# pabloconrat/our_first_climate_model

Measured on NVIDIA B200. Metric: column*wavelength*layer flux updates/s (repwvl-100 RCE step), higher is better.
Workload: dtype f64

## Files before the change

our_first_climate_model_b200/csrc/rcm_capi.cu:

```cuda
#include <algorithm>
#include <cmath>
#include <cstdio>
#include <cstdlib>
#include <cstring>
#include <new>
#include <functional>
#include <string>
#include <vector>

#include "rcm_jac.cuh"
#include "rcm_fdh.cuh"
#include "rcm_lbl_diag.cuh"

#ifndef M_PI
#define M_PI 3.14159265358979323846
#endif

struct rcm_solver {
    int device = 0;
    cudaStream_t own_stream = nullptr, stream = nullptr;
    rcm_params p{};
    DevConst dc{};
    bool const_dirty = true;
    int opt_angle_cubes = 1;
// ... 421 lines not shown
}


bool use_split(const rcm_solver* s) {
    return !s->lbl_mode && s->has_table && s->nactive == 5 && s->opt_config == 0 && s->opt_path == 0;
}

struct SplitGeom { int ntiles, nitem, nsplit; };
SplitGeom split_geom(const rcm_solver* s, int ncols) {
    SplitGeom g;
    g.ntiles = (ncols + 15) / 16;
    g.nitem = (s->dc.nwvl + 3) / 4;
    g.nsplit = (g.nitem + rcm_split_ipu() - 1) / rcm_split_ipu();
    return g;
}

int ensure_split(rcm_solver* s) {
    const SplitGeom g = split_geom(s, s->cap);
    const size_t tiles = (size_t)g.ntiles, need_part = tiles * g.nsplit * rcm_split_part_doubles();
    if (tiles > s->tile_cap || !s->d_tile) {
        CU(dalloc(s->d_tile, tiles * rcm_split_tile_bytes()));
        s->tile_cap = tiles;
        s->tile_vmr_valid = false;
    }
    if (need_part > s->spart_cap || !s->d_spart) {
        CU(dalloc(s->d_spart, need_part));
        s->spart_cap = need_part;
    }
    if (tiles > s->multi_cap || !s->d_multi) {
        if (s->d_multi) CU(cudaFree(s->d_multi));
        s->d_multi = nullptr;
        CU(cudaMalloc((void**)&s->d_multi, 2 * tiles * sizeof(unsigned)));
        s->multi_cap = tiles;
    }
    if (!s->d_dTstat) CU(dalloc(s->d_dTstat, (size_t)s->cap));
    if (!s->d_counter) {
        CU(dalloc(s->d_counter, (size_t)4));
        CU(cudaMemsetAsync(s->d_counter, 0, 4 * sizeof(unsigned), s->stream));
    }
    return RCM_OK;
}

SplitArgs split_args(rcm_solver* s, int col0, int ncols, int which) {
    const SplitGeom g = split_geom(s, ncols);
    const size_t o = (size_t)col0, t0 = o / 16;
    SplitArgs a{};
    a.ncol = ncols;
    a.diag_ncol = s->ncol;
    a.ntiles = g.ntiles;
    a.nsplit = g.nsplit;
    a.ipu = rcm_split_ipu();
    a.nitem = g.nitem;
    a.nunits = g.ntiles * g.nsplit;
    a.stage_rows = s->opt_stage_rows;
    a.clampk = s->clampk;
    a.h2o_slot = s->h2o_slot;
    a.tau_clamp = s->tau_clamp;
    a.T_floor = s->T_floor;
    a.coef = s->d_coef3;
    a.planck_c = s->d_planck_c;
    a.planck_k = s->d_planck_k;
    a.exp_tab = s->d_exp_tab;
    a.Tlayer = s->d_T + o * NLAY;
    a.Tsurf = s->d_Ts + o;
    a.vmr = s->d_vmr + o * s->nactive * NLAY;
    a.rel_hum = s->d_rh + o * NLAY;
    a.Tprev = s->d_Tprev + o * NLAY;
    a.time_h = s->d_time + o;
    a.E_down = s->d_Ed + o * NLEV;
    a.E_up = s->d_Eu + o * NLEV;
    a.dE = s->d_dE + o * NLAY;
    a.dt = s->d_dt + o;
    a.diag = s->d_diag + o * 4;
    a.solar_col = s->has_col_solar ? s->d_solar_col + o : nullptr;
    a.cloud_col = s->has_col_cloud ? s->d_cloud_col + o : nullptr;
    a.tile = s->d_tile + t0 * rcm_split_tile_bytes();
    a.part = s->d_spart + t0 * g.nsplit * rcm_split_part_doubles();
    a.dTstat = s->d_dTstat + o;
    a.counter = s->d_counter + which;
    a.quota = 1 << 30;
    return a;
}

int split_grid(const rcm_solver* s, const SplitArgs& a, int nsm) {
    (void)s;
    if (a.quota < a.nunits) return (a.nunits + a.quota - 1) / a.quota;
    int per_sm = 3;
    if (const char* e = std::getenv("RCM_CTAS_PER_SM")) {
        const int v = std::atoi(e);
        if (v >= 1 && v < per_sm) per_sm = v;
    }
    return std::min(a.nunits, nsm * per_sm);
}

int split_rt(rcm_solver* s, const SplitArgs& a, int nsm, cudaStream_t st, bool timed) {
    std::pair<cudaEvent_t, cudaEvent_t> ev{};
    if (timed) {
        if (!s->ev_free.empty()) {
            ev = s->ev_free.back();
            s->ev_free.pop_back();
        } else {
            CU(cudaEventCreate(&ev.first));
            CU(cudaEventCreate(&ev.second));
        }
        CU(cudaEventRecord(ev.first, st));
    }
    CU(rcm_launch_split_rt(a, split_grid(s, a, nsm), st));
    s->launches += 1;
    if (timed) {
        CU(cudaEventRecord(ev.second, st));
        s->ev_used.push_back(ev);
        if (s->ev_used.size() >= 1024) {
            const int rc = rcm_kernel_time_ms(s, 0, nullptr, nullptr);
            if (rc != RCM_OK) return rc;
        }
    }
    return RCM_OK;
}

int split_advance(rcm_solver* s, int nsteps) {
    int st = refresh_const(s);
    if (st != RCM_OK) return st;
    st = ensure_split(s);
    if (st != RCM_OK) return st;
    const int nsm = nsm_of(s);
    const SplitArgs a = split_args(s, 0, s->ncol, 0);
    SplitColFlags f{};
    f.prep = 1;
    f.first = (s->step_index == 0);
    f.write_all_vmr = !s->tile_vmr_valid;
    CU(rcm_launch_split_col(a, f, s->stream));
    s->launches += 1;
    s->tile_vmr_valid = true;
    static const int multi_rounds = std::getenv("RCM_MULTI_ROUNDS") ? std::atoi(std::getenv("RCM_MULTI_ROUNDS")) : 24;
    const int grid1 = split_grid(s, a, nsm);
    const bool few_rounds = a.nunits < (long long)multi_rounds * grid1;
    const bool fits = (long long)a.nunits * nsteps + 2LL * grid1 < (1LL << 31);
    if (nsteps >= 2 && fits && (s->opt_multi == 2 || (s->opt_multi == 1 && few_rounds))) {
        SplitMultiArgs m{};
        m.nsteps = nsteps;
        m.done = s->d_multi;
        m.ready = s->d_multi + a.ntiles;
        CU(cudaMemsetAsync(s->d_multi, 0, 2 * (size_t)a.ntiles * sizeof(unsigned), s->stream));
        SplitArgs am = a;
        am.quota = 1 << 30;
        CU(rcm_launch_split_multi(am, m, split_grid(s, am, nsm), s->stream));
        s->launches += 1;
        return RCM_OK;
    }
    for (int k = 0; k < nsteps; ++k) {
        st = split_rt(s, a, nsm, s->stream, k < 4);
        if (st != RCM_OK) return st;
        SplitColFlags e{};
        e.finish = 1;
        e.prep = (k + 1 < nsteps);
        e.first = 0;
        e.write_out = (k + 1 == nsteps);
        e.diag_step = k;
        CU(rcm_launch_split_col(a, e, s->stream));
        s->launches += 1;
    }
    return RCM_OK;
}

int launch(rcm_solver* s, int mode, int nsteps, bool want_diag) {
    int st = refresh_const(s);
    if (st != RCM_OK) return st;
    if (mode == MODE_RT ? !s->has_spectral : !s->has_table) return fail(s, RCM_ERR_STATE, "no lookup table loaded");
    if (s->ncol <= 0) return fail(s, RCM_ERR_STATE, "no columns loaded");
    const int nsm = nsm_of(s);
    Part parts[2];
    const int nparts = plan_parts(s, s->ncol, nsm, parts);
    std::pair<cudaEvent_t, cudaEvent_t> ev;
    if (!s->ev_free.empty()) {
        ev = s->ev_free.back();
        s->ev_free.pop_back();
    } else {
        CU(cudaEventCreate(&ev.first));
        CU(cudaEventCreate(&ev.second));
    }
    CU(cudaEventRecord(ev.first, s->stream));
    for (int ip = 0; ip < nparts; ++ip) {
        st = launch_part(s, mode, nsteps, want_diag, parts[ip], nsm, s->stream);
        if (st != RCM_OK) return st;
    }
    CU(cudaEventRecord(ev.second, s->stream));
    if (mode == MODE_STEP) s->ev_used.push_back(ev); else s->ev_free.push_back(ev);
    if (s->ev_used.size() >= 1024) {
        st = rcm_kernel_time_ms(s, 0, nullptr, nullptr);
        if (st != RCM_OK) return st;
    }
    return RCM_OK;
}


int step_host_split(rcm_solver* s, int nchunk, const double* Tlayer_in, const double* Tsurf_in, const double* vmr_active_in,
                    double* E_down, double* E_up, double* dE, double* Tlayer_out, double* Tsurf_out) {
    int st = ensure_split(s);
    if (st != RCM_OK) return st;
    if (!s->sp_up) {
        int lo = 0, hi = 0;
        CU(cudaDeviceGetStreamPriorityRange(&lo, &hi));
        CU(cudaStreamCreateWithPriority(&s->sp_up, cudaStreamNonBlocking, hi));
        CU(cudaStreamCreateWithPriority(&s->sp_down, cudaStreamNonBlocking, hi));
        for (int i = 0; i < 2; ++i) CU(cudaStreamCreateWithPriority(&s->sp_rt[i], cudaStreamNonBlocking, lo));
        for (int i = 0; i < 24; ++i) {
            CU(cudaEventCreateWithFlags(&s->sp_prep[i], cudaEventDisableTiming));
            CU(cudaEventCreateWithFlags(&s->sp_rtdone[i], cudaEventDisableTiming));
        }
        CU(cudaEventCreateWithFlags(&s->sp_end, cudaEventDisableTiming));
    }
    const int nsm = nsm_of(s);
    const int per = ((s->ncol + nchunk - 1) / nchunk + 15) / 16 * 16;
    int bounds[24];
    int nb = 0;
    bounds[nb++] = 0;
    if (nchunk >= 4 && per >= 64) {
        const int q = per / 4 / 16 * 16;
        bounds[nb++] = q;
        for (int c0 = per; c0 < s->ncol - q; c0 += per) bounds[nb++] = c0;
        bounds[nb++] = std::max(bounds[nb - 1], s->ncol - q) / 16 * 16;
    } else {
        for (int c0 = per; c0 < s->ncol; c0 += per) bounds[nb++] = c0;
    }
    bounds[nb] = s->ncol;
    const size_t D = sizeof(double);
    const int na = s->nactive;
    auto enqueue = [&](bool timed) -> int {
    int nk = 0;
// ... 1510 lines not shown
```

our_first_climate_model_b200/csrc/rcm_kernels.cu:

```cuda
#include <cfloat>
#include <cstdio>

#include "rcm_kernels.cuh"
#include "rcm_diag.cuh"
#include "rcm_jac.cuh"
#include "rcm_fjac.cuh"
#include "rcm_fdh.cuh"
#include "rcm_lbl_diag.cuh"

__constant__ DevConst cst;

cudaError_t rcm_upload_const(const DevConst& c) { return cudaMemcpyToSymbol(cst, &c, sizeof(DevConst)); }

namespace {

#include "rcm_device_math.cuh"
#include "rcm_step_kernel.cuh"

__global__ void rcm_coef_kernel(const double* __restrict__ src, double* __restrict__ dst, int nt, int ns, int nw,
                                int np, int nact, const int* __restrict__ species) {
    const size_t n = (size_t)NLAY * (nt - 1) * nw * nact;
    for (size_t i = blockIdx.x * (size_t)blockDim.x + threadIdx.x; i < n; i += (size_t)gridDim.x * blockDim.x) {
        size_t r = i;
        const int k = r % nact; r /= nact;
// ... 156 lines not shown
    for (int k = 0; k < a.doublings; ++k) {
        const double denom = sub(1.0, mul(r, r));
        const double r2 = add(r, dvd(mul(mul(r, t), t), denom));
        const double t2 = dvd(mul(t, t), denom);
        const double s2 = add(dvd(add(mul(t, s_dir), mul(mul(mul(t_dir, r_dir), r), t)), denom), mul(t_dir, s_dir));
        const double rd2 = add(dvd(add(mul(mul(t, s_dir), r), mul(mul(t, t_dir), r)), denom), r_dir);
        t_dir = mul(t_dir, t_dir);
        s_dir = s2;
        r_dir = rd2;
        r = r2;
        t = t2;
    }
    const double r_total = add(r_dir, mul(mul(dvd(add(t_dir, s_dir), sub(1.0, mul(albedo, r))), t), albedo));
    if (a.r_total) a.r_total[i] = r_total;
    if (a.solar_irr) a.solar_irr[i] = mul(mul(mul(a.daytime, a.E_0), mu_s), sub(1.0, r_total));
    if (a.cloud_tau) a.cloud_tau[i] = dvd(tau_s, 2.0);
}

__global__ void __launch_bounds__(256) rcm_cplkavg_kernel(int n, const double* lo, const double* hi, const double* t,
                                                          double* out, const double* tab, int narrow) {
    __shared__ double stab[EXP_TAB * EXP_REP];
    for (int i = threadIdx.x; i < EXP_TAB * EXP_REP; i += blockDim.x) stab[i] = tab[i / EXP_REP];
    __syncthreads();
    const unsigned tl = (unsigned)__cvta_generic_to_shared(stab + (threadIdx.x & (EXP_REP - 1)));
    for (int i = blockIdx.x * blockDim.x + threadIdx.x; i < n; i += gridDim.x * blockDim.x)
    {
        const double whi = 1.0E7 / lo[i], wlo = 1.0E7 / hi[i];
        const bool bin_ok = whi > wlo && wlo >= 0. && (whi - wlo) / whi < 1.e-2;
        out[i] = narrow ? cplkavg_narrow(lo[i], hi[i], whi, wlo, bin_ok, t[i], tl) : cplkavg_dev(lo[i], hi[i], t[i]);
    }
}

}

size_t rcm_step_smem_bytes(int C, int nactive, int nthreads) {
#define RCM_SHAPE(CC, TT) \
    if (C == CC && nthreads == TT) return nactive == 5 ? Smem<CC, TT, 5>::bytes(5) : Smem<CC, TT, 0>::bytes(nactive);
    RCM_SHAPE(16, 128)
    RCM_SHAPE(8, 128)
    RCM_SHAPE(4, 128)
    RCM_SHAPE(32, 192)
    RCM_SHAPE(16, 96)
#undef RCM_SHAPE
    return 0;
}

template <int MODE, int NACT, int C, int NT>
static cudaError_t launch_t(const StepArgs& a, int nactive, int grid, cudaStream_t st) {
    const size_t smem = Smem<C, NT, NACT>::bytes(nactive);
    auto kern = a.clampk ? rcm_step_kernel<MODE, NACT, C, NT, true> : rcm_step_kernel<MODE, NACT, C, NT, false>;
    cudaError_t e = cudaFuncSetAttribute(kern, cudaFuncAttributeMaxDynamicSharedMemorySize, (int)smem);
    if (e != cudaSuccess) return e;
    kern<<<grid, NT, smem, st>>>(a);
    return cudaGetLastError();
}

template <int MODE>
static cudaError_t launch_m(const StepArgs& a, int nactive, int grid, cudaStream_t st) {
    const bool five = (nactive == 5);
#define RCM_SHAPE(CC, TT)                  \
    if (a.C == CC && a.nthreads == TT)     \
        return five ? launch_t<MODE, 5, CC, TT>(a, nactive, grid, st) : launch_t<MODE, 0, CC, TT>(a, nactive, grid, st);
    RCM_SHAPE(16, 128)
    RCM_SHAPE(8, 128)
    RCM_SHAPE(4, 128)
    RCM_SHAPE(32, 192)
    RCM_SHAPE(16, 96)
#undef RCM_SHAPE
    return cudaErrorInvalidValue;
}

cudaError_t rcm_launch_step(int mode, const StepArgs& a, int nactive, int grid, cudaStream_t st) {
    switch (mode) {
        case MODE_STEP: return launch_m<MODE_STEP>(a, nactive, grid, st);
        case MODE_TAU: return launch_m<MODE_TAU>(a, nactive, grid, st);
        case MODE_RT: return launch_m<MODE_RT>(a, nactive, grid, st);
    }
    return cudaErrorInvalidValue;
}

size_t rcm_split_tile_bytes() { return TILE_BYTES; }
size_t rcm_split_part_doubles() { return SPLIT_PART; }
int rcm_split_ipu() { return SPLIT_IPU; }

cudaError_t rcm_launch_split_col(const SplitArgs& a, const SplitColFlags& f, cudaStream_t st) {
    rcm_split_col_kernel<<<a.ntiles, SPLIT_COL_NT, 0, st>>>(a, f);
    return cudaGetLastError();
}

cudaError_t rcm_launch_split_rt(const SplitArgs& a, int grid, cudaStream_t st) {
    auto kern = a.clampk ? rcm_split_rt_kernel<true> : rcm_split_rt_kernel<false>;
    cudaError_t e = cudaFuncSetAttribute(kern, cudaFuncAttributeMaxDynamicSharedMemorySize, (int)SPLIT_SMEM);
    if (e != cudaSuccess) return e;
    kern<<<grid, SPLIT_NT, SPLIT_SMEM, st>>>(a);
    return cudaGetLastError();
}

cudaError_t rcm_launch_split_multi(const SplitArgs& a, const SplitMultiArgs& m, int grid, cudaStream_t st) {
    auto kern = a.clampk ? rcm_split_multi_kernel<true> : rcm_split_multi_kernel<false>;
    cudaError_t e = cudaFuncSetAttribute(kern, cudaFuncAttributeMaxDynamicSharedMemorySize, (int)SPLIT_SMEM);
    if (e != cudaSuccess) return e;
    kern<<<grid, SPLIT_NT, SPLIT_SMEM, st>>>(a, m);
    return cudaGetLastError();
}

size_t rcm_reduce_scratch_doubles(int nsteps) { return (size_t)nsteps * RED_BLOCKS * 4; }

cudaError_t rcm_launch_reduce_diag(const double* diag, int nsteps, int ncol, double dT_converged, double* scratch,
                                   unsigned* ticket, double* scalars, cudaStream_t st) {
    rcm_reduce_diag_kernel<<<dim3(RED_BLOCKS, nsteps), RED_THREADS, 0, st>>>(diag, ncol, dT_converged, scratch, ticket, scalars);
    return cudaGetLastError();
}

cudaError_t rcm_launch_coef(const double* xsec_file, double* coef, int nt, int ns, int nw, int np, int nact,
                            const int* d_species, cudaStream_t st) {
    rcm_coef_kernel<<<296, 256, 0, st>>>(xsec_file, coef, nt, ns, nw, np, nact, d_species);
    return cudaGetLastError();
}

cudaError_t rcm_launch_coef3(const double* coef4, double* coef3, size_t nrows, cudaStream_t st) {
    rcm_coef3_kernel<<<296, 256, 0, st>>>(coef4, coef3, nrows);
    return cudaGetLastError();
}

cudaError_t rcm_launch_microbench(int which, double* out, const double* tab, long iters, int grid,
                                  cudaStream_t st) {
    switch (which) {
        case 0: rcm_microbench_kernel<0><<<grid, 256, 0, st>>>(out, iters, tab); break;
        case 1: rcm_microbench_kernel<1><<<grid, 256, 0, st>>>(out, iters, tab); break;
        case 2: rcm_microbench_kernel<2><<<grid, 256, 0, st>>>(out, iters, tab); break;
        case 3: rcm_microbench_kernel<3><<<grid, 256, 0, st>>>(out, iters, tab); break;
        default: return cudaErrorInvalidValue;
    }
    return cudaGetLastError();
}

cudaError_t rcm_launch_solar(const SolarArgs& a, cudaStream_t st) {
    if (a.n <= 0) return cudaSuccess;
    rcm_solar_kernel<<<(a.n + 127) / 128, 128, 0, st>>>(a);
    return cudaGetLastError();
}

cudaError_t rcm_launch_cplkavg(int n, const double* lo, const double* hi, const double* t, double* out,
                               const double* exp_tab, int narrow, cudaStream_t st) {
    rcm_cplkavg_kernel<<<148, 256, 0, st>>>(n, lo, hi, t, out, exp_tab, narrow);
    return cudaGetLastError();
}

size_t rcm_lbl_smem_bytes(int C, int nthreads) {
    return ((size_t)EXP_TAB * EXP_REP + (size_t)TBD_LEN * 3 + 2 * C + (size_t)HALF * nthreads +
            (size_t)NLEV * (nthreads / 2)) * sizeof(double);
}

cudaError_t rcm_launch_lbl_prep(const LblArgs& a, cudaStream_t st) {
    rcm_lbl_prep_kernel<<<(a.ncol + 127) / 128, 128, 0, st>>>(a);
    return cudaGetLastError();
}

cudaError_t rcm_launch_lbl_rt(const LblArgs& a, cudaStream_t st, cudaEvent_t ev0, cudaEvent_t ev1) {
    constexpr int C = RCM_LBL_C, NT = RCM_LBL_NT;
    const size_t smem = rcm_lbl_smem_bytes(C, NT);
    auto kern = a.clampk ? rcm_lbl_rt_kernel<C, NT, true> : rcm_lbl_rt_kernel<C, NT, false>;
    cudaError_t e = cudaFuncSetAttribute(kern, cudaFuncAttributeMaxDynamicSharedMemorySize, (int)smem);
    if (e != cudaSuccess) return e;
    if (ev0) cudaEventRecord(ev0, st);
    kern<<<a.ntiles * a.nchunks, NT, smem, st>>>(a);
    if (ev1) cudaEventRecord(ev1, st);
    return cudaGetLastError();
}

cudaError_t rcm_launch_lbl_finish(const LblArgs& a, cudaStream_t st) {
    rcm_lbl_finish_kernel<<<a.ncol, LBL_FIN_NT, 0, st>>>(a);
    return cudaGetLastError();
}

cudaError_t rcm_launch_lbl_step(const LblArgs& a, cudaStream_t st, cudaEvent_t ev0, cudaEvent_t ev1) {
    cudaError_t e = rcm_launch_lbl_prep(a, st);
// ... 97 lines not shown
```

our_first_climate_model_b200/csrc/rcm_kernels.cuh:

```cuda
#ifndef RCM_KERNELS_CUH
#define RCM_KERNELS_CUH

#include <cuda_runtime.h>

#include "rcm_internal.h"

constexpr int NLAY = RCM_NLAYER;
constexpr int NLEV = RCM_NLEVEL;
constexpr int MAX_ANGLE = 64;
constexpr int MAX_TPERT = 16;
constexpr int PLK_MAX = 128;
constexpr int MAX_PAIR = 16;
constexpr int HALF = NLAY / 2;
constexpr int RCM_LBL_C = 16, RCM_LBL_NT = 128;
#ifndef RCM_EXP_LOG2
#define RCM_EXP_LOG2 10
#endif
constexpr int EXP_LOG2 = RCM_EXP_LOG2, EXP_TAB = 1 << EXP_LOG2;
constexpr int EXP_REP = (EXP_LOG2 == 7) ? 8 : 1;
#ifdef RCM_EXP_DEG_OVERRIDE
constexpr int EXP_DEG = RCM_EXP_DEG_OVERRIDE;
#else
constexpr int EXP_DEG = (EXP_LOG2 == 7) ? 3 : 2;
#endif
// ... 33 lines not shown
    double tau_clamp;
    double T_floor;
    int ntiles;
    int nsteps;
    long step_index;
    const double* __restrict__ coef;
    const double* __restrict__ planck_c;
    const double* __restrict__ planck_k;
    double* Tlayer;
    double* Tsurf;
    double* vmr;
    const double* rel_hum;
    double* Tprev;
    float* time_h;
    double* E_down;
    double* E_up;
    double* dE;
    double* dt;
    double* diag;
    double* tau_io;
    int* lowpos_t;
    const double* exp_tab;
    int h2o_slot;
    const double* solar_col;
    const double* cloud_col;
};

struct LblArgs {
    int ncol, ntiles, nwvl, nchunks, chunk_len, nact, h2o_slot, o3_slot;
    int clampk;
    long step_index;
    double co2_factor, tau_clamp;
    const double* __restrict__ wvl_lo;
    const double* __restrict__ wvl_hi;
    const double* __restrict__ wn_hi;
    const double* __restrict__ wn_lo;
    const int* __restrict__ bin_ok;
    const double* __restrict__ tau3;
    const double* __restrict__ h2o_ref;
    const double* __restrict__ o3_ref;
    const double* __restrict__ exp_tab;
    double* Tlayer; double* Tsurf; double* vmr; const double* rel_hum; double* Tprev; float* time_h;
    double* sH; double* sO; double* dTstat;
    double* part;
    double* E_down; double* E_up; double* dE; double* dt; double* diag;
    const double* solar_col; const double* cloud_col;
};

struct SplitArgs {
    int ncol;
    int diag_ncol;
    int ntiles, nsplit, ipu, nitem, nunits;
    int stage_rows, clampk, h2o_slot;
    double tau_clamp, T_floor;
    const double* __restrict__ coef;
    const double* __restrict__ planck_c;
    const double* __restrict__ planck_k;
    const double* __restrict__ exp_tab;
    double* Tlayer; double* Tsurf; double* vmr; const double* rel_hum; double* Tprev; float* time_h;
    double* E_down; double* E_up; double* dE; double* dt; double* diag;
    const double* solar_col; const double* cloud_col;
    unsigned char* tile;
    double* part;
    double* dTstat;
    unsigned* counter;
    int quota;
};
struct SplitColFlags {
    int finish;
    int prep;
    int first;
    int write_all_vmr;
    int write_out;
    int diag_step;
};
struct SplitMultiArgs {
    int nsteps;
    unsigned* done;
    unsigned* ready;
};
size_t rcm_split_tile_bytes();
size_t rcm_split_part_doubles();
int rcm_split_ipu();
cudaError_t rcm_launch_split_col(const SplitArgs& a, const SplitColFlags& f, cudaStream_t st);
cudaError_t rcm_launch_split_rt(const SplitArgs& a, int grid, cudaStream_t st);
cudaError_t rcm_launch_split_multi(const SplitArgs& a, const SplitMultiArgs& m, int grid, cudaStream_t st);

enum { MODE_STEP = 0, MODE_TAU = 1, MODE_RT = 2 };

size_t rcm_step_smem_bytes(int C, int nactive, int nthreads);
cudaError_t rcm_upload_const(const DevConst& c);
cudaError_t rcm_launch_step(int mode, const StepArgs& a, int nactive, int grid, cudaStream_t st);
size_t rcm_reduce_scratch_doubles(int nsteps);
cudaError_t rcm_launch_reduce_diag(const double* diag, int nsteps, int ncol, double dT_converged, double* scratch,
                                   unsigned* ticket, double* scalars, cudaStream_t st);
cudaError_t rcm_launch_coef(const double* xsec_file, double* coef, int nt, int ns, int nw, int np, int nact,
                            const int* d_species, cudaStream_t st);
cudaError_t rcm_launch_coef3(const double* coef4, double* coef3, size_t nrows, cudaStream_t st);
cudaError_t rcm_launch_microbench(int which, double* out, const double* tab, long iters, int grid,
                                  cudaStream_t st);
size_t rcm_lbl_smem_bytes(int C, int nthreads);
cudaError_t rcm_launch_lbl_step(const LblArgs& a, cudaStream_t st, cudaEvent_t ev0, cudaEvent_t ev1);
struct SolarArgs {
    int n, doublings;
    double tau_s, mu_s, g_asym, albedo, daytime, E_0;
    const double* tau_s_col; const double* mu_s_col; const double* albedo_col;
    double* solar_irr; double* r_total; double* cloud_tau;
};
cudaError_t rcm_launch_solar(const SolarArgs& a, cudaStream_t st);
cudaError_t rcm_launch_cplkavg(int n, const double* lo, const double* hi, const double* t, double* out,
                               const double* exp_tab, int narrow, cudaStream_t st);

#endif
```

our_first_climate_model_b200/csrc/rcm_split_kernels.cuh:

```cuda
#pragma once

constexpr int SPLIT_C = 16, SPLIT_NT = 128, SPLIT_G = 4;
constexpr int SPLIT_IPU = 5;
constexpr int SPLIT_COL_NT = 128;

constexpr int TB_INVT = 0;
constexpr int TB_DELT = TB_INVT + TBD_LEN;
constexpr int TB_DTDP = TB_DELT + TBD_LEN;
constexpr int TB_VMR = TB_DTDP + TBD_LEN;
constexpr int TB_INVTS = TB_VMR + 5 * TBD_LEN;
constexpr int TB_CLOUD = TB_INVTS + SPLIT_C;
constexpr int TB_DOUBLES = TB_CLOUD + SPLIT_C;
constexpr int TBI_IT = 0;
constexpr int TBI_ROWSEL = TBI_IT + TBI_LEN;
constexpr int TBI_ROWOFF = TBI_ROWSEL + TBI_LEN;
constexpr int TBI_OUTSIDE = TBI_ROWOFF + NLAY * NCAND;
constexpr int TB_INTS = (TBI_OUTSIDE + 1 + 3) / 4 * 4;
constexpr int TILE_BYTES = TB_DOUBLES * 8 + TB_INTS * 4;
static_assert(TILE_BYTES % 16 == 0, "bulk copies move multiples of 16 bytes");
constexpr int ROWB3 = 16 * 8;
constexpr int ROWS3 = ROWB3 + 16;
constexpr int ROWBUF3 = NLAY * NCAND * ROWS3;
constexpr int SPLIT_PART = 2 * NLEV * SPLIT_C;

// ... 203 lines not shown

__device__ __forceinline__ unsigned ld_acquire_gpu(const unsigned* p) {
    unsigned v;
    asm volatile("ld.acquire.gpu.global.u32 %0, [%1];" : "=r"(v) : "l"(p) : "memory");
    return v;
}
__device__ __forceinline__ void st_release_gpu(unsigned* p, unsigned v) {
    asm volatile("st.release.gpu.global.u32 [%0], %1;" ::"l"(p), "r"(v) : "memory");
}

__device__ __noinline__ void wait_tile_ready(const unsigned* flag, unsigned step) {
    unsigned spins = 0;
    while (ld_acquire_gpu(flag) < step) {
        __nanosleep(128);
        if (++spins > (1u << 23)) __trap();
    }
    asm volatile("fence.proxy.async;" ::: "memory");
}

__device__ __forceinline__ void mbar_init(unsigned mbar, unsigned count) {
    asm volatile("mbarrier.init.shared::cta.b64 [%0], %1;" ::"r"(mbar), "r"(count) : "memory");
    asm volatile("fence.mbarrier_init.release.cluster;" ::: "memory");
}
__device__ __forceinline__ void tma_load_1d(unsigned dst, const void* src, unsigned bytes, unsigned mbar) {
    asm volatile("fence.proxy.async.shared::cta;" ::: "memory");
    asm volatile("mbarrier.arrive.expect_tx.shared::cta.b64 _, [%0], %1;" ::"r"(mbar), "r"(bytes) : "memory");
    asm volatile("cp.async.bulk.shared::cluster.global.mbarrier::complete_tx::bytes [%0], [%1], %2, [%3];" ::"r"(dst), "l"(src),
                 "r"(bytes), "r"(mbar)
                 : "memory");
}
__device__ __forceinline__ void mbar_wait(unsigned mbar, unsigned phase) {
    asm volatile(
        "{\n\t.reg .pred p;\n\t"
        "WAIT_%=:\n\t"
        "mbarrier.try_wait.parity.shared::cta.b64 p, [%0], %1;\n\t"
        "@p bra DONE_%=;\n\t"
        "bra WAIT_%=;\n\t"
        "DONE_%=:\n\t}" ::"r"(mbar),
        "r"(phase)
        : "memory");
}

__device__ __forceinline__ double tau_k1(const double* tb, int s, int r, const double2* cf, double cl) {
    const double dT = tb[TB_DELT + s], dTdP = tb[TB_DTDP + s];
    double c[16];
#pragma unroll
    for (int q2 = 0; q2 < 8; ++q2) {
        const double2 v = cf[q2];
        c[2 * q2] = v.x;
        c[2 * q2 + 1] = v.y;
    }
    double acc = 0.0;
#pragma unroll
    for (int k = 0; k < 5; ++k) {
        double v = fma(c[3 * k + 1], dT, c[3 * k]);
        v = fma(c[3 * k + 2], dTdP, v);
        acc = fma(v, tb[TB_VMR + k * TBD_LEN + s], acc);
    }
    acc = acc * cst.numDens[r];
    return fma(cst.cloud_w[r], cl, acc);
}

__device__ __forceinline__ double planck_b(double pc, double pk, double invT, unsigned tab_lane) {
    return div_fast(pk, exp_scaled<false>(pc, invT, tab_lane) - 1.0);
}

__device__ __forceinline__ void load_exp_tab(double* s_exp, const double* tab, int tid, int nt) {
    for (int i = tid; i < EXP_TAB * EXP_REP; i += nt) s_exp[i] = tab[i / EXP_REP];
}

__device__ __forceinline__ void load_tile(double* tb, const unsigned char* tile, int tid, int nt) {
    const uint4* src = reinterpret_cast<const uint4*>(tile);
    uint4* dst = reinterpret_cast<uint4*>(tb);
    for (int i = tid; i < TILE_BYTES / 16; i += nt) dst[i] = src[i];
}

constexpr size_t SPLIT_SMEM = (size_t)EXP_TAB * EXP_REP * 8 + (size_t)SPLIT_G * ROWBUF3 + TILE_BYTES + 2 * PLK_MAX * 8 + 48;
static_assert(SPLIT_PART * 8 <= ROWBUF3, "a warp's row buffer carries its partial fluxes after the wavelength loop");

static_assert(sizeof(SplitColSmem) <= (size_t)SPLIT_G * ROWBUF3, "the K5 body of the multi-step kernel works in the row buffers");
static_assert(SPLIT_COL_NT == SPLIT_NT, "the multi-step kernel runs the K5 body with its own CTA");

template <bool CLAMPK>
__global__ void __launch_bounds__(SPLIT_NT, 3) rcm_split_rt_kernel(const SplitArgs a) {
#define RCM_SPLIT_MULTI 0
#include "rcm_split_unit_loop.inc"
#undef RCM_SPLIT_MULTI
}

template <bool CLAMPK>
__global__ void __launch_bounds__(SPLIT_NT, 3) rcm_split_multi_kernel(const __grid_constant__ SplitArgs a, const __grid_constant__ SplitMultiArgs m) {
#define RCM_SPLIT_MULTI 1
#include "rcm_split_unit_loop.inc"
#undef RCM_SPLIT_MULTI
}
```

our_first_climate_model_b200/csrc/rcm_split_unit_loop.inc:

```
    constexpr int C = SPLIT_C, NT = SPLIT_NT, G = SPLIT_G;
    extern __shared__ __align__(128) unsigned char smem_raw[];
    double* const s_exp = reinterpret_cast<double*>(smem_raw);
    unsigned char* const s_rows = smem_raw + (size_t)EXP_TAB * EXP_REP * 8;
    double* const tb = reinterpret_cast<double*>(s_rows + (size_t)G * ROWBUF3);
    const int* const tbi = reinterpret_cast<const int*>(tb + TB_DOUBLES);
    double* const s_plk = reinterpret_cast<double*>(reinterpret_cast<unsigned char*>(tb) + TILE_BYTES);
    unsigned long long* const s_mbar = reinterpret_cast<unsigned long long*>(s_plk + 2 * PLK_MAX);
    volatile int* const s_next = reinterpret_cast<volatile int*>(s_mbar + 1);

    const int tid = threadIdx.x, lane = tid & 31, warp = tid >> 5;
    const int h = tid & 1, q = tid >> 1, c = q % C, g = q / C;
    const int sb = tbd(h * HALF, c), sbi = tbix(h * HALF, c);
    const int nwvl = cst.nwvl;
    load_exp_tab(s_exp, a.exp_tab, tid, NT);
    const unsigned tab_lane = (unsigned)__cvta_generic_to_shared(s_exp + (lane & (EXP_REP - 1)));
    const bool plk_smem = nwvl <= PLK_MAX;
    if (plk_smem)
        for (int i = tid; i < nwvl; i += NT) {
            s_plk[i] = a.planck_c[i];
            s_plk[PLK_MAX + i] = a.planck_k[i];
        }
    const unsigned mbar = (unsigned)__cvta_generic_to_shared(s_mbar);
    const unsigned tb_addr = (unsigned)__cvta_generic_to_shared(tb);
    unsigned char* const rows = s_rows + (size_t)warp * ROWBUF3;
    const unsigned rows_addr = (unsigned)__cvta_generic_to_shared(rows);
#if RCM_SPLIT_MULTI
    auto fetch_block = [&](int u) {
        const int tile_u = (u % a.nunits) / a.nsplit;
        const bool ready = ld_acquire_gpu(m.ready + tile_u) >= (unsigned)(u / a.nunits);
        s_next[2] = !ready;
        if (!ready) return;
        asm volatile("fence.proxy.async;" ::: "memory");
        tma_load_1d(tb_addr, a.tile + (size_t)tile_u * TILE_BYTES, TILE_BYTES, mbar);
    };
    if (tid == 0) {
        mbar_init(mbar, 1);
        const int u = (int)atomicAdd(a.counter, 1u);
        s_next[0] = u;
        s_next[1] = 1;
        s_next[2] = 0;
        if (u < a.nunits * m.nsteps) fetch_block(u);
    }
#else
    if (tid == 0) {
        mbar_init(mbar, 1);
        const int u = (int)atomicAdd(a.counter, 1u);
        s_next[0] = u;
        s_next[1] = 1;
        if (u < a.nunits) tma_load_1d(tb_addr, a.tile + (size_t)(u / a.nsplit) * TILE_BYTES, TILE_BYTES, mbar);
    }
#endif
    __syncthreads();
    int unit = *s_next;
    unsigned phase = 0;

    auto request_rows = [&](int w) {
        __syncwarp();
        const char* base = reinterpret_cast<const char*>(a.coef) + (size_t)w * ROWB3 + (lane & 7) * 16;
        const unsigned dst0 = rows_addr + (lane & 7) * 16 + (lane >> 3) * ROWS3;
        const int* ro = tbi + TBI_ROWOFF + (lane >> 3);
        unsigned off[NCAND * NLAY / 4];
#pragma unroll
        for (int i = 0; i < NCAND * NLAY / 4; ++i) off[i] = (unsigned)ro[4 * i];
#pragma unroll
        for (int i = 0; i < NCAND * NLAY / 4; ++i) cp_async16(dst0 + 4 * i * ROWS3, base + off[i]);
        cp_async_commit();
    };
    const int tau_clamp_hi = __double2hiint(a.tau_clamp);
#if RCM_SPLIT_MULTI
    while (unit < a.nunits * m.nsteps) {
        const int step = unit / a.nunits, unit_s = unit - step * a.nunits;
        const int tile = unit_s / a.nsplit, split = unit_s - tile * a.nsplit;
        if (tid == 0) {
            s_next[4] = tile;
            s_next[5] = step;
            s_next[6] = unit_s;
        }
#else
    while (unit < a.nunits) {
        const int tile = unit / a.nsplit, split = unit - tile * a.nsplit;
#endif
        mbar_wait(mbar, phase);
        phase ^= 1u;
        const bool staged = a.stage_rows && !tbi[TBI_OUTSIDE];
        const int item0 = split * a.ipu, item1 = min(item0 + a.ipu, a.nitem);
        double E1[HALF], E2[HALF], Eu20 = 0.0;
#pragma unroll
        for (int j = 0; j < HALF; ++j) E1[j] = E2[j] = 0.0;
        if (staged) request_rows(min(g + item0 * G, nwvl - 1));
#pragma unroll 1
        for (int item = item0; item < item1; ++item) {
            const int w_any = g + item * G;
            const bool real = w_any < nwvl;
            const int w = real ? w_any : nwvl - 1;
            double tau[HALF], Bo[HALF];
            const double cl = tb[TB_CLOUD + c];
            if (staged) {
                cp_async_wait_all();
                __syncwarp();
#pragma unroll
                for (int j = 0; j < HALF; ++j) {
                    const double v = tau_k1(tb, sb + j * C, h * HALF + j,
                                            reinterpret_cast<const double2*>(rows + tbi[TBI_ROWSEL + sbi + j * C]), cl);
                    tau[j] = CLAMPK ? v : clamp_hi(v, tau_clamp_hi);
                }
                if (item + 1 < item1) request_rows(min(w_any + G, nwvl - 1));
            } else {
#pragma unroll
                for (int j = 0; j < HALF; ++j) {
                    const int cell = cst.ipcell[h * HALF + j] + tbi[TBI_IT + sbi + j * C];
                    const double v = tau_k1(tb, sb + j * C, h * HALF + j,
                                            reinterpret_cast<const double2*>(a.coef) + (size_t)(cell * nwvl + w) * 8, cl);
                    tau[j] = fmax(CLAMPK ? v : clamp_hi(v, tau_clamp_hi), TAU_FLOOR);
                }
            }
            const double pc = plk_smem ? s_plk[w] : __ldg(a.planck_c + w);
            const double pk = !real ? 0.0 : plk_smem ? s_plk[PLK_MAX + w] : __ldg(a.planck_k + w);
#pragma unroll
            for (int j = 0; j < HALF; ++j) Bo[j] = planck_b(pc, pk, tb[TB_INVT + sb + j * C], tab_lane);
            const double Bs = planck_b(pc, pk, tb[TB_INVTS + c], tab_lane);
            sweep_item<CLAMPK>(tau, Bo, Bs, h, tab_lane, E1, E2, Eu20);
        }
        {
            double* part = reinterpret_cast<double*>(s_rows + (size_t)g * ROWBUF3);
#pragma unroll
            for (int j = 0; j < HALF; ++j) {
                const int l = h ? (NLAY - 1 - j) : j;
                part[l * C + c] = h ? E2[j] : E1[j];
                part[(NLEV + l) * C + c] = h ? E1[j] : E2[j];
            }
            if (h) part[(NLEV + NLAY) * C + c] = Eu20;
        }
        __syncthreads();
        if (tid == 0) {
            const int taken = s_next[1];
#if RCM_SPLIT_MULTI
            const int u = (int)atomicAdd(a.counter, 1u);
            s_next[0] = u;
            s_next[1] = taken + 1;
            if (u < a.nunits * m.nsteps) fetch_block(u);
        }
        double* out = a.part + (size_t)s_next[6] * SPLIT_PART;
#else
            const int u = (taken < a.quota) ? (int)atomicAdd(a.counter, 1u) : a.nunits;
            s_next[0] = u;
            s_next[1] = taken + 1;
            if (u < a.nunits) tma_load_1d(tb_addr, a.tile + (size_t)(u / a.nsplit) * TILE_BYTES, TILE_BYTES, mbar);
        }
        double* out = a.part + (size_t)unit * SPLIT_PART;
#endif
        for (int i = tid; i < SPLIT_PART; i += NT) {
            double sum = 0.0;
            if (i / C != NLAY) {
#pragma unroll
                for (int gg = 0; gg < G; ++gg) sum += reinterpret_cast<const double*>(s_rows + (size_t)gg * ROWBUF3)[i];
            }
            out[i] = sum;
        }
#if RCM_SPLIT_MULTI
        {
            __threadfence();
            __syncthreads();
            const int tile_e = s_next[4], step_e = s_next[5];
            if (tid == 0) {
                const unsigned before = atomicAdd(m.done + tile_e, 1u);
                s_next[3] = ((before + 1u) % (unsigned)a.nsplit) == 0u;
            }
            __syncthreads();
            if (s_next[3]) {
                __threadfence();
                SplitColFlags f;
                f.finish = 1;
                f.prep = (step_e + 1 < m.nsteps);
                f.first = 0;
                f.write_all_vmr = 0;
                f.write_out = (step_e + 1 == m.nsteps);
                f.diag_step = step_e;
                split_col_body_call(a, f, tile_e, *reinterpret_cast<SplitColSmem*>(s_rows));
                __threadfence();
                __syncthreads();
                if (tid == 0) st_release_gpu(m.ready + tile_e, (unsigned)(step_e + 1));
            }
            if (tid == 0 && s_next[2]) {
                const int u = s_next[0], tile_u = (u % a.nunits) / a.nsplit;
                wait_tile_ready(m.ready + tile_u, (unsigned)(u / a.nunits));
                tma_load_1d(tb_addr, a.tile + (size_t)tile_u * TILE_BYTES, TILE_BYTES, mbar);
            }
        }
#endif
        __syncthreads();
        unit = *s_next;
    }
```

Baseline: 40.21 billion.

## Warp-specialize split RT kernel into producer and consumer warps with smem ring

Rewrites the per-step split radiative-transfer kernel as a warp-specialized design. Producer warps (registers lowered via setmaxnreg) compute optical depth and Planck terms into a double-buffered shared-memory ring guarded by mbarriers. Consumer warps (registers raised) run the flux sweep and write partial sums. The goal is to overlap coefficient gathering and tau computation with the sweep, and to relieve register pressure on the sweep. In exchange it doubles threads per CTA, drops from 3 to 2 CTAs per SM, and adds mbarrier and named-barrier handshakes. The multi-step kernel keeps the old loop.

```diff
diff --git a/our_first_climate_model_b200/csrc/rcm_capi.cu b/our_first_climate_model_b200/csrc/rcm_capi.cu
--- a/our_first_climate_model_b200/csrc/rcm_capi.cu
+++ b/our_first_climate_model_b200/csrc/rcm_capi.cu
@@ -527,10 +527,9 @@
     return a;
 }
 
-int split_grid(const rcm_solver* s, const SplitArgs& a, int nsm) {
+int split_grid(const rcm_solver* s, const SplitArgs& a, int nsm, int per_sm) {
     (void)s;
     if (a.quota < a.nunits) return (a.nunits + a.quota - 1) / a.quota;
-    int per_sm = 3;
     if (const char* e = std::getenv("RCM_CTAS_PER_SM")) {
         const int v = std::atoi(e);
         if (v >= 1 && v < per_sm) per_sm = v;
@@ -550,7 +549,7 @@
         }
         CU(cudaEventRecord(ev.first, st));
     }
-    CU(rcm_launch_split_rt(a, split_grid(s, a, nsm), st));
+    CU(rcm_launch_split_rt(a, split_grid(s, a, nsm, rcm_split_rt_ctas_per_sm()), st));
     s->launches += 1;
     if (timed) {
         CU(cudaEventRecord(ev.second, st));
@@ -578,7 +577,7 @@
     s->launches += 1;
     s->tile_vmr_valid = true;
     static const int multi_rounds = std::getenv("RCM_MULTI_ROUNDS") ? std::atoi(std::getenv("RCM_MULTI_ROUNDS")) : 24;
-    const int grid1 = split_grid(s, a, nsm);
+    const int grid1 = split_grid(s, a, nsm, 3);
     const bool few_rounds = a.nunits < (long long)multi_rounds * grid1;
     const bool fits = (long long)a.nunits * nsteps + 2LL * grid1 < (1LL << 31);
     if (nsteps >= 2 && fits && (s->opt_multi == 2 || (s->opt_multi == 1 && few_rounds))) {
@@ -589,7 +588,7 @@
         CU(cudaMemsetAsync(s->d_multi, 0, 2 * (size_t)a.ntiles * sizeof(unsigned), s->stream));
         SplitArgs am = a;
         am.quota = 1 << 30;
-        CU(rcm_launch_split_multi(am, m, split_grid(s, am, nsm), s->stream));
+        CU(rcm_launch_split_multi(am, m, split_grid(s, am, nsm, 3), s->stream));
         s->launches += 1;
         return RCM_OK;
     }
diff --git a/our_first_climate_model_b200/csrc/rcm_kernels.cu b/our_first_climate_model_b200/csrc/rcm_kernels.cu
--- a/our_first_climate_model_b200/csrc/rcm_kernels.cu
+++ b/our_first_climate_model_b200/csrc/rcm_kernels.cu
@@ -262,6 +262,7 @@
 size_t rcm_split_tile_bytes() { return TILE_BYTES; }
 size_t rcm_split_part_doubles() { return SPLIT_PART; }
 int rcm_split_ipu() { return SPLIT_IPU; }
+int rcm_split_rt_ctas_per_sm() { return SPLIT_WS_CTAS; }
 
 cudaError_t rcm_launch_split_col(const SplitArgs& a, const SplitColFlags& f, cudaStream_t st) {
     rcm_split_col_kernel<<<a.ntiles, SPLIT_COL_NT, 0, st>>>(a, f);
@@ -270,9 +271,9 @@
 
 cudaError_t rcm_launch_split_rt(const SplitArgs& a, int grid, cudaStream_t st) {
     auto kern = a.clampk ? rcm_split_rt_kernel<true> : rcm_split_rt_kernel<false>;
-    cudaError_t e = cudaFuncSetAttribute(kern, cudaFuncAttributeMaxDynamicSharedMemorySize, (int)SPLIT_SMEM);
-    if (e != cudaSuccess) return e;
-    kern<<<grid, SPLIT_NT, SPLIT_SMEM, st>>>(a);
+    cudaError_t e = cudaFuncSetAttribute(kern, cudaFuncAttributeMaxDynamicSharedMemorySize, (int)SPLIT_WS_SMEM);
+    if (e != cudaSuccess) return e;
+    kern<<<grid, SPLIT_WS_NT, SPLIT_WS_SMEM, st>>>(a);
     return cudaGetLastError();
 }
 
diff --git a/our_first_climate_model_b200/csrc/rcm_kernels.cuh b/our_first_climate_model_b200/csrc/rcm_kernels.cuh
--- a/our_first_climate_model_b200/csrc/rcm_kernels.cuh
+++ b/our_first_climate_model_b200/csrc/rcm_kernels.cuh
@@ -139,6 +139,7 @@
 size_t rcm_split_tile_bytes();
 size_t rcm_split_part_doubles();
 int rcm_split_ipu();
+int rcm_split_rt_ctas_per_sm();
 cudaError_t rcm_launch_split_col(const SplitArgs& a, const SplitColFlags& f, cudaStream_t st);
 cudaError_t rcm_launch_split_rt(const SplitArgs& a, int grid, cudaStream_t st);
 cudaError_t rcm_launch_split_multi(const SplitArgs& a, const SplitMultiArgs& m, int grid, cudaStream_t st);
diff --git a/our_first_climate_model_b200/csrc/rcm_split_kernels.cuh b/our_first_climate_model_b200/csrc/rcm_split_kernels.cuh
--- a/our_first_climate_model_b200/csrc/rcm_split_kernels.cuh
+++ b/our_first_climate_model_b200/csrc/rcm_split_kernels.cuh
@@ -309,15 +309,200 @@
 static_assert(SPLIT_COL_NT == SPLIT_NT, "the multi-step kernel runs the K5 body with its own CTA");
 
 template <bool CLAMPK>
-__global__ void __launch_bounds__(SPLIT_NT, 3) rcm_split_rt_kernel(const SplitArgs a) {
-#define RCM_SPLIT_MULTI 0
+__global__ void __launch_bounds__(SPLIT_NT, 3) rcm_split_multi_kernel(const __grid_constant__ SplitArgs a, const __grid_constant__ SplitMultiArgs m) {
 #include "rcm_split_unit_loop.inc"
-#undef RCM_SPLIT_MULTI
+}
+
+constexpr int SPLIT_WS_NT = 2 * SPLIT_NT;
+constexpr int SPLIT_WS_CTAS = 2;
+constexpr int SPLIT_PROD_REGS = 64, SPLIT_CONS_REGS = 192;
+static_assert((SPLIT_PROD_REGS + SPLIT_CONS_REGS) * SPLIT_NT * SPLIT_WS_CTAS == 65536, "setmaxnreg moves registers, it adds none");
+constexpr int SPLIT_RING = 2;
+constexpr int RING_TAU = 0, RING_B = TBD_LEN, RING_BS = 2 * TBD_LEN, RING_DOUBLES = 2 * TBD_LEN + SPLIT_C;
+static_assert(RING_DOUBLES >= SPLIT_PART, "the slot of a unit's last round carries the group's partial fluxes");
+constexpr int SPLIT_WS_MBARS = 1 + 2 * SPLIT_G * SPLIT_RING;
+constexpr size_t SPLIT_WS_SMEM = (size_t)EXP_TAB * EXP_REP * 8 + (size_t)SPLIT_G * ROWBUF3 + TILE_BYTES +
+                                 (size_t)SPLIT_G * SPLIT_RING * RING_DOUBLES * 8 + 2 * PLK_MAX * 8 + SPLIT_WS_MBARS * 8 +
+                                 (2 + SPLIT_G * SPLIT_RING) * 4;
+static_assert(SPLIT_WS_CTAS * (SPLIT_WS_SMEM + 1024) <= 228 * 1024, "two CTAs per SM");
+
+__device__ __forceinline__ void mbar_arrive(unsigned mbar) {
+    asm volatile("mbarrier.arrive.shared::cta.b64 _, [%0];" ::"r"(mbar) : "memory");
+}
+__device__ __forceinline__ void named_bar_sync(int id, int nthreads) {
+    asm volatile("bar.sync %0, %1;" ::"r"(id), "r"(nthreads) : "memory");
 }
 
 template <bool CLAMPK>
-__global__ void __launch_bounds__(SPLIT_NT, 3) rcm_split_multi_kernel(const __grid_constant__ SplitArgs a, const __grid_constant__ SplitMultiArgs m) {
-#define RCM_SPLIT_MULTI 1
-#include "rcm_split_unit_loop.inc"
-#undef RCM_SPLIT_MULTI
-}
+__global__ void __launch_bounds__(SPLIT_WS_NT, SPLIT_WS_CTAS) rcm_split_rt_kernel(const SplitArgs a) {
+    constexpr int C = SPLIT_C, NT = SPLIT_NT, G = SPLIT_G, R = SPLIT_RING;
+    extern __shared__ __align__(128) unsigned char smem_raw[];
+    double* const s_exp = reinterpret_cast<double*>(smem_raw);
+    unsigned char* const s_rows = smem_raw + (size_t)EXP_TAB * EXP_REP * 8;
+    double* const tb = reinterpret_cast<double*>(s_rows + (size_t)G * ROWBUF3);
+    const int* const tbi = reinterpret_cast<const int*>(tb + TB_DOUBLES);
+    double* const s_ring = reinterpret_cast<double*>(reinterpret_cast<unsigned char*>(tb) + TILE_BYTES);
+    double* const s_plk = s_ring + G * R * RING_DOUBLES;
+    unsigned long long* const s_mbar = reinterpret_cast<unsigned long long*>(s_plk + 2 * PLK_MAX);
+    volatile int* const s_next = reinterpret_cast<volatile int*>(s_mbar + SPLIT_WS_MBARS);
+    volatile int* const s_hdr = s_next + 2;
+
+    const int tid = threadIdx.x, lane = tid & 31, warp = __shfl_sync(0xffffffffu, tid >> 5, 0);
+    const int h = lane & 1, c = lane >> 1, g = warp % G;
+    const int sb = tbd(h * HALF, c);
+    const int nwvl = cst.nwvl;
+    load_exp_tab(s_exp, a.exp_tab, tid, SPLIT_WS_NT);
+    const unsigned tab_lane = (unsigned)__cvta_generic_to_shared(s_exp + (lane & (EXP_REP - 1)));
+    const bool plk_smem = nwvl <= PLK_MAX;
+    if (plk_smem)
+        for (int i = tid; i < nwvl; i += SPLIT_WS_NT) {
+            s_plk[i] = a.planck_c[i];
+            s_plk[PLK_MAX + i] = a.planck_k[i];
+        }
+    const unsigned mbar = (unsigned)__cvta_generic_to_shared(s_mbar);
+    const unsigned tb_addr = (unsigned)__cvta_generic_to_shared(tb);
+    const unsigned full0 = mbar + 8 * (1 + g * R), empty0 = mbar + 8 * (1 + G * R + g * R);
+    double* const ring = s_ring + g * R * RING_DOUBLES;
+    if (tid == 0) {
+        mbar_init(mbar, 1);
+        for (int i = 1; i < SPLIT_WS_MBARS; ++i) mbar_init(mbar + 8 * i, 32);
+        const int u = (int)atomicAdd(a.counter, 1u);
+        s_next[0] = u;
+        s_next[1] = 1;
+        if (u < a.nunits) tma_load_1d(tb_addr, a.tile + (size_t)(u / a.nsplit) * TILE_BYTES, TILE_BYTES, mbar);
+    }
+    __syncthreads();
+    unsigned k = 0;
+
+    if (warp < G) {
+        asm volatile("setmaxnreg.dec.sync.aligned.u32 %0;" ::"n"(SPLIT_PROD_REGS));
+        const int sbi = tbix(h * HALF, c);
+        const unsigned rows_addr = (unsigned)__cvta_generic_to_shared(s_rows + (size_t)g * ROWBUF3);
+        const unsigned char* const rows = s_rows + (size_t)g * ROWBUF3;
+        auto request_rows = [&](int w) {
+            __syncwarp();
+            const char* base = reinterpret_cast<const char*>(a.coef) + (size_t)w * ROWB3 + (lane & 7) * 16;
+            const unsigned dst0 = rows_addr + (lane & 7) * 16 + (lane >> 3) * ROWS3;
+            const int* ro = tbi + TBI_ROWOFF + (lane >> 3);
+#pragma unroll
+            for (int i = 0; i < NCAND * NLAY / 4; ++i) cp_async16(dst0 + 4 * i * ROWS3, base + (unsigned)ro[4 * i]);
+            cp_async_commit();
+        };
+        const int tau_clamp_hi = __double2hiint(a.tau_clamp);
+        int unit = s_next[0];
+        unsigned phase = 0;
+        while (unit < a.nunits) {
+            const int split = unit % a.nsplit;
+            mbar_wait(mbar, phase);
+            phase ^= 1u;
+            const bool staged = a.stage_rows && !tbi[TBI_OUTSIDE];
+            const int item0 = split * a.ipu, item1 = min(item0 + a.ipu, a.nitem);
+            if (staged) request_rows(min(g + item0 * G, nwvl - 1));
+#pragma unroll 1
+            for (int item = item0; item < item1; ++item, ++k) {
+                const int w_any = g + item * G;
+                const bool real = w_any < nwvl;
+                const int w = real ? w_any : nwvl - 1;
+                const int slot = k % R;
+                double* const out = ring + slot * RING_DOUBLES;
+                const double cl = tb[TB_CLOUD + c];
+                mbar_wait(empty0 + 8 * slot, ((k / R) & 1) ^ 1);
+                if (staged) {
+                    cp_async_wait_all();
+                    __syncwarp();
+#pragma unroll
+                    for (int j = 0; j < HALF; ++j) {
+                        const double v = tau_k1(tb, sb + j * C, h * HALF + j,
+                                                reinterpret_cast<const double2*>(rows + tbi[TBI_ROWSEL + sbi + j * C]), cl);
+                        out[RING_TAU + sb + j * C] = CLAMPK ? v : clamp_hi(v, tau_clamp_hi);
+                    }
+                    if (item + 1 < item1) request_rows(min(w_any + G, nwvl - 1));
+                } else {
+#pragma unroll
+                    for (int j = 0; j < HALF; ++j) {
+                        const int cell = cst.ipcell[h * HALF + j] + tbi[TBI_IT + sbi + j * C];
+                        const double v = tau_k1(tb, sb + j * C, h * HALF + j,
+                                                reinterpret_cast<const double2*>(a.coef) + (size_t)(cell * nwvl + w) * 8, cl);
+                        out[RING_TAU + sb + j * C] = fmax(CLAMPK ? v : clamp_hi(v, tau_clamp_hi), TAU_FLOOR);
+                    }
+                }
+                const double pc = plk_smem ? s_plk[w] : __ldg(a.planck_c + w);
+                const double pk = !real ? 0.0 : plk_smem ? s_plk[PLK_MAX + w] : __ldg(a.planck_k + w);
+#pragma unroll
+                for (int j = 0; j < HALF; ++j) out[RING_B + sb + j * C] = planck_b(pc, pk, tb[TB_INVT + sb + j * C], tab_lane);
+                out[RING_BS + c] = planck_b(pc, pk, tb[TB_INVTS + c], tab_lane);
+                if (lane == 0) s_hdr[g * R + slot] = unit;
+                mbar_arrive(full0 + 8 * slot);
+            }
+            named_bar_sync(1, NT);
+            if (tid == 0) {
+                const int taken = s_next[1];
+                const int u = (taken < a.quota) ? (int)atomicAdd(a.counter, 1u) : a.nunits;
+                s_next[0] = u;
+                s_next[1] = taken + 1;
+                if (u < a.nunits) tma_load_1d(tb_addr, a.tile + (size_t)(u / a.nsplit) * TILE_BYTES, TILE_BYTES, mbar);
+            }
+            named_bar_sync(1, NT);
+            unit = s_next[0];
+        }
+        const int slot = k % R;
+        mbar_wait(empty0 + 8 * slot, ((k / R) & 1) ^ 1);
+        if (lane == 0) s_hdr[g * R + slot] = a.nunits;
+        mbar_arrive(full0 + 8 * slot);
+    } else {
+        asm volatile("setmaxnreg.inc.sync.aligned.u32 %0;" ::"n"(SPLIT_CONS_REGS));
+        const int ct = tid - NT;
+        while (true) {
+            int slot = k % R;
+            mbar_wait(full0 + 8 * slot, (k / R) & 1);
+            const int unit = __shfl_sync(0xffffffffu, s_hdr[g * R + slot], 0);
+            if (unit >= a.nunits) break;
+            const int split = unit % a.nsplit;
+            const int item0 = split * a.ipu, nround = min(item0 + a.ipu, a.nitem) - item0;
+            double E1[HALF], E2[HALF], Eu20 = 0.0;
+#pragma unroll
+            for (int j = 0; j < HALF; ++j) E1[j] = E2[j] = 0.0;
+#pragma unroll 1
+            for (int r = 1;; ++r) {
+                const double* const in = ring + slot * RING_DOUBLES;
+                double tau[HALF], Bo[HALF];
+#pragma unroll
+                for (int j = 0; j < HALF; ++j) {
+                    tau[j] = in[RING_TAU + sb + j * C];
+                    Bo[j] = in[RING_B + sb + j * C];
+                }
+                const double Bs = in[RING_BS + c];
+                if (r < nround) mbar_arrive(empty0 + 8 * slot);
+                sweep_item<CLAMPK>(tau, Bo, Bs, h, tab_lane, E1, E2, Eu20);
+                if (r == nround) break;
+                ++k;
+                slot = k % R;
+                mbar_wait(full0 + 8 * slot, (k / R) & 1);
+            }
+            __syncwarp();
+            {
+                double* part = ring + slot * RING_DOUBLES;
+#pragma unroll
+                for (int j = 0; j < HALF; ++j) {
+                    const int l = h ? (NLAY - 1 - j) : j;
+                    part[l * C + c] = h ? E2[j] : E1[j];
+                    part[(NLEV + l) * C + c] = h ? E1[j] : E2[j];
+                }
+                if (h) part[(NLEV + NLAY) * C + c] = Eu20;
+            }
+            named_bar_sync(2, NT);
+            double* out = a.part + (size_t)unit * SPLIT_PART;
+            for (int i = ct; i < SPLIT_PART; i += NT) {
+                double sum = 0.0;
+                if (i / C != NLAY) {
+#pragma unroll
+                    for (int gg = 0; gg < G; ++gg) sum += s_ring[(gg * R + slot) * RING_DOUBLES + i];
+                }
+                out[i] = sum;
+            }
+            named_bar_sync(2, NT);
+            mbar_arrive(empty0 + 8 * slot);
+            ++k;
+        }
+    }
+}
diff --git a/our_first_climate_model_b200/csrc/rcm_split_unit_loop.inc b/our_first_climate_model_b200/csrc/rcm_split_unit_loop.inc
--- a/our_first_climate_model_b200/csrc/rcm_split_unit_loop.inc
+++ b/our_first_climate_model_b200/csrc/rcm_split_unit_loop.inc
@@ -24,7 +24,6 @@
     const unsigned tb_addr = (unsigned)__cvta_generic_to_shared(tb);
     unsigned char* const rows = s_rows + (size_t)warp * ROWBUF3;
     const unsigned rows_addr = (unsigned)__cvta_generic_to_shared(rows);
-#if RCM_SPLIT_MULTI
     auto fetch_block = [&](int u) {
         const int tile_u = (u % a.nunits) / a.nsplit;
         const bool ready = ld_acquire_gpu(m.ready + tile_u) >= (unsigned)(u / a.nunits);
@@ -41,15 +40,6 @@
         s_next[2] = 0;
         if (u < a.nunits * m.nsteps) fetch_block(u);
     }
-#else
-    if (tid == 0) {
-        mbar_init(mbar, 1);
-        const int u = (int)atomicAdd(a.counter, 1u);
-        s_next[0] = u;
-        s_next[1] = 1;
-        if (u < a.nunits) tma_load_1d(tb_addr, a.tile + (size_t)(u / a.nsplit) * TILE_BYTES, TILE_BYTES, mbar);
-    }
-#endif
     __syncthreads();
     int unit = *s_next;
     unsigned phase = 0;
@@ -67,7 +57,6 @@
         cp_async_commit();
     };
     const int tau_clamp_hi = __double2hiint(a.tau_clamp);
-#if RCM_SPLIT_MULTI
     while (unit < a.nunits * m.nsteps) {
         const int step = unit / a.nunits, unit_s = unit - step * a.nunits;
         const int tile = unit_s / a.nsplit, split = unit_s - tile * a.nsplit;
@@ -76,10 +65,6 @@
             s_next[5] = step;
             s_next[6] = unit_s;
         }
-#else
-    while (unit < a.nunits) {
-        const int tile = unit / a.nsplit, split = unit - tile * a.nsplit;
-#endif
         mbar_wait(mbar, phase);
         phase ^= 1u;
         const bool staged = a.stage_rows && !tbi[TBI_OUTSIDE];
@@ -134,21 +119,12 @@
         __syncthreads();
         if (tid == 0) {
             const int taken = s_next[1];
-#if RCM_SPLIT_MULTI
             const int u = (int)atomicAdd(a.counter, 1u);
             s_next[0] = u;
             s_next[1] = taken + 1;
             if (u < a.nunits * m.nsteps) fetch_block(u);
         }
         double* out = a.part + (size_t)s_next[6] * SPLIT_PART;
-#else
-            const int u = (taken < a.quota) ? (int)atomicAdd(a.counter, 1u) : a.nunits;
-            s_next[0] = u;
-            s_next[1] = taken + 1;
-            if (u < a.nunits) tma_load_1d(tb_addr, a.tile + (size_t)(u / a.nsplit) * TILE_BYTES, TILE_BYTES, mbar);
-        }
-        double* out = a.part + (size_t)unit * SPLIT_PART;
-#endif
         for (int i = tid; i < SPLIT_PART; i += NT) {
             double sum = 0.0;
             if (i / C != NLAY) {
@@ -157,7 +133,6 @@
             }
             out[i] = sum;
         }
-#if RCM_SPLIT_MULTI
         {
             __threadfence();
             __syncthreads();
@@ -187,7 +162,6 @@
                 tma_load_1d(tb_addr, a.tile + (size_t)tile_u * TILE_BYTES, TILE_BYTES, mbar);
             }
         }
-#endif
         __syncthreads();
         unit = *s_next;
     }
```

Result: slower. 39.52 billion (median of 6 runs) (-1.7%).
